# QuantEcon/dynamic_factor_models

Hardware: AMD Instinct MI355X
Metric: Kalman-smoother passes/sec, N=200 T=500 r=8 panel (higher is better)
Workload: dtype f64; 1 GPU; BASELINE configs[1]: synthetic panel N=200 T=500 r=8, batch=1024 replicates per GPU, one full Kalman-smoother pass per step, balanced; N=200, T=500, r=8, batch_per_gpu=1024, global_batch=1024, mode=pass, parallelism=replicate-sharded x1

## Files before the change

dynamic_factor_models_amd/csrc/dfm_cov8.h:

```cpp
#pragma once
#include "dfm_cov.h"
#include "dfm_grid.h"

namespace dfm {

constexpr int kCov8TileDoubles = 8 * kTileStride<8>;
constexpr int kCov8ScratchDoubles = 5 * kCov8TileDoubles + 64;
constexpr int kCov8Keep = 8;

struct Cov8Dst {
    double* tab;
    int tab_cap;
    double* tab_over;
    double* stead;
    double* PT;
    double* xi0;
    double* llc;
    int* E;
    int* fill;
    double* PsInf;
    double* SP11; double* SU; double* P0s;
};

template <int R, int NLEV, int KEEP>
__device__ __forceinline__ void cov_grid(const FastArgs& a, int b, double Cel, double ldfull, double* wsm, const Cov8Dst& o,
                                         Grid<R>& G) {
    constexpr int TS = kTileStride<R>, RR = R * R, RT = R * kTileStride<R>;
    const int lane = G.l, i = G.i, j = G.j;
    double* L0 = wsm;
    double* L1 = L0 + RT;
    double* LPT = L1 + RT;
    double* LJ = LPT + RT;
    const int T = a.T, r = a.r;
    const bool diag = (i == j);
    const size_t mo = (size_t)b * RR + lane;

    const double Ael = a.A[mo];
    double Qi = a.Q[mo];
    double Omf = a.P0[mo];
    const double mu0c = a.mu0[(size_t)b * R + j];
    const double detQ = G.sweep_inverse(Qi);
    const double detP0 = G.sweep_inverse(Omf);
    L0[TS * i + j] = Qi;
    L1[TS * j + i] = Ael;
    G.sync();
    const double PsiT = dot_rows<R>(L0, L1, i, j);
    G.sync();
    LPT[TS * i + j] = PsiT;
    L0[TS * j + i] = PsiT;
    G.sync();
    const double Phi = dot_rows<R>(L0, L1, i, j);
    double q0;
    {
        const double xi0r = G.sum_j(Omf * mu0c);
        if (j == 0) o.xi0[i] = xi0r;
        double part = diag ? mu0c * xi0r : 0.0;
        part = G.sum_j(part);
        q0 = G.sum_i(part);
    }
    G.sync();

    LogProd detprod;
    double detM_last = 1.0;
    int E = 0;
    double Zk[KEEP], Jk[KEEP];
#pragma unroll
    for (int u = 0; u < KEEP; ++u) { Zk[u] = 0.0; Jk[u] = 0.0; }
    double Zlast = 0.0, Jlast = 0.0, Glast = 0.0;
    for (int e = 0;; ++e) {
        double Z = Omf + Phi;
        const double detM = G.sweep_inverse(Z);
        L0[TS * i + j] = Z;
        G.sync();
        const double Jr = dot_rows<R>(L0, LPT, i, j);
        L1[TS * j + i] = Jr;
        G.sync();
        const double tmp = dot_rows<R>(LPT, L1, i, j);
        const double Gm = dot_rows<R>(LPT, L0, i, j);
        const double Omf_new = (Qi - tmp) + Cel;
        const bool gsame = G.all_true(close_enough(Omf_new, Omf));
        double* te = (e < o.tab_cap ? o.tab : o.tab_over) + (size_t)e * 3 * RR;
        te[lane] = Z; te[RR + lane] = Jr; te[2 * RR + lane] = Gm;
#pragma unroll
        for (int u = 0; u < KEEP; ++u) {
            Zk[u] = (u == e) ? Z : Zk[u];
            Jk[u] = (u == e) ? Jr : Jk[u];
        }
        Zlast = Z; Jlast = Jr; Glast = Gm;
        E = e + 1;
        detprod.mul(detM);
        detM_last = detM;
        Omf = Omf_new;
        G.sync();
        if (gsame || e + 1 >= T) break;
    }
    const int ts = E - 1;

    double Ps = Omf;
    const double detOmT = G.sweep_inverse(Ps);
    o.PT[lane] = Ps;
    if (lane == 0) {
        const double sum_ldz = -(detprod.log_value() + (double)(T - E) * log(detM_last));
        const double LD = log(detOmT) + log(detP0) + (double)T * log(detQ) - sum_ldz;
        o.llc[0] = (double)a.N * (double)T * kLog2PiF + (double)T * ldfull + LD + q0;
        o.E[0] = E;
    }

    const int npr = r * (r + 1) / 2;
    const bool pout = a.P_smooth != nullptr && i < r && j <= i;
    double* prow = a.P_smooth ? a.P_smooth + (size_t)b * T * npr + i * (i + 1) / 2 + j : nullptr;
    auto emit = [&](int trow, double P) { if (pout) prow[(size_t)trow * npr] = P; };
    emit(T - 1, Ps);
    double SP = Ps, SU = 0.0;
    int fill_lo = 0, fill_hi = 0;
    int t = T - 1, cur_e = -2;
    double Zc = 0.0, Jc = 0.0;
    while (t >= 0) {
        const int e = t < ts ? t : ts;
        if (e != cur_e) {
            if (e == ts) {
                Zc = Zlast; Jc = Jlast;
            } else if (e < KEEP) {
#pragma unroll
                for (int u = 0; u < KEEP; ++u) {
                    Zc = (u == e) ? Zk[u] : Zc;
                    Jc = (u == e) ? Jk[u] : Jc;
                }
            } else {
                const double* te = (e < o.tab_cap ? o.tab : o.tab_over) + (size_t)e * 3 * RR;
                Zc = te[lane]; Jc = te[RR + lane];
            }
            cur_e = e;
            LJ[TS * i + j] = Jc;
        }
        L0[TS * i + j] = Ps;
        G.sync();
        const double U = dot_rows<R>(L0, LJ, i, j);
        L1[TS * j + i] = U;
        G.sync();
        const double Psn = Zc + dot_rows<R>(LJ, L1, i, j);
        const bool gsame = G.all_true(close_enough(Psn, Ps));
        const bool skip = (e == ts && t > ts && gsame);
        const int plo = ts >= 1 ? ts : 1;
        const double cu = skip ? (double)(t - ts + 1) : 1.0;
        const double cp = (t >= 1 ? 1.0 : 0.0) + (skip ? (double)(t - plo) : 0.0);
        SU = fma(cu, U, SU);
        SP = fma(cp, Psn, SP);
        if (t >= 1) emit(t - 1, Psn);
        if ((t == 0 || (skip && ts == 0)) && o.P0s) o.P0s[lane] = Psn;
        if (skip) {
            o.PsInf[lane] = Psn;
            fill_lo = plo - 1;
            fill_hi = t - 1;
            t = ts - 1;
        } else {
            t -= 1;
        }
        Ps = Psn;
        G.sync();
    }
    if (lane == 0) { o.fill[0] = fill_lo; o.fill[1] = fill_hi; }
    if (o.SP11) { o.SP11[lane] = SP; o.SU[lane] = SU; }

    {
        const double Zs = Zlast, Js = Jlast, Gs = Glast;
        o.stead[lane] = Zs;
        o.stead[2 * RR + lane] = Gs;
        o.stead[1 * RR + lane] = Js;
        double MG = Gs, MJ = Js;
        auto square2 = [&]() {
            L0[TS * i + j] = MG;
            L1[TS * j + i] = MG;
            LPT[TS * i + j] = MJ;
            LJ[TS * j + i] = MJ;
            G.sync();
            MG = dot_rows<R>(L0, L1, i, j);
            MJ = dot_rows<R>(LPT, LJ, i, j);
            G.sync();
        };
        for (int l = 1; l < a.L; l <<= 1) square2();
#pragma unroll 1
        for (int k = 0; k < NLEV; ++k) {
            o.stead[(3 + k) * RR + lane] = MG;
            o.stead[(3 + NLEV + k) * RR + lane] = MJ;
            if (k + 1 < NLEV) square2();
        }
    }
}

template <int NLEV>
__device__ __forceinline__ void cov_wave8(const FastArgs& a, int b, double Cel, double ldfull, double* wsm, const Cov8Dst& o,
                                          int lane) {
    Grid<8> G;
    G.l = lane; G.i = lane >> 3; G.j = lane & 7; G.prow = nullptr; G.red = nullptr; G.tt = nullptr;
    cov_grid<8, NLEV, kCov8Keep>(a, b, Cel, ldfull, wsm, o, G);
}

template <int NDR>
__device__ __forceinline__ double gram_wave8(const double* __restrict__ Lg, const double* __restrict__ Rg, int N, int lane,
                                             double* Cs) {
    constexpr int R = 8;
    double W[NDR][2][R];
    bool own[NDR][2];
    double ld = 0.0;
#pragma unroll
    for (int q = 0; q < NDR; ++q)
#pragma unroll
        for (int e = 0; e < 2; ++e) {
            const int c = 2 * lane + 128 * q + e;
            own[q][e] = c < N;
            const int cc = own[q][e] ? c : N - 1;
            const double rv = own[q][e] ? Rg[cc] : 1.0;
            const double ri = own[q][e] ? 1.0 / rv : 0.0;
            ld += log(rv);
#pragma unroll
            for (int k = 0; k < R; ++k) W[q][e][k] = Lg[(size_t)cc * R + k] * ri;
        }
    c_chunk<R, NDR, 0, 18, true>(W, Lg, own, lane, Cs);
    c_chunk<R, NDR, 18, 18, true>(W, Lg, own, lane, Cs);
    return wave_allsum(ld);
}

}
```

dynamic_factor_models_amd/csrc/pass_fused.hip:

```cpp
#include <stdlib.h>
#include <string.h>

#include <type_traits>

#include "dfm_cov8.h"
#include "dfm_gram.h"
#include "dfm_kernels.h"
#include "dfm_scan.h"

#ifndef DFM_DMA_MOD
#define DFM_DMA_MOD ""
#endif

namespace dfm {

namespace {

using lds_char_ptr_f = __attribute__((address_space(3))) char*;

__device__ __forceinline__ void dma16f(const void* gsrc, unsigned lds_dst, bool nt) {
    unsigned keep;
    if (nt) {
        asm volatile(
            "s_mov_b32 %0, m0\n\t"
            "s_mov_b32 m0, %2\n\t"
            "s_nop 0\n\t"
            "global_load_lds_dwordx4 %1, off nt\n\t"
            "s_mov_b32 m0, %0"
            : "=&s"(keep)
            : "v"(gsrc), "s"(lds_dst)
            : "memory");
    } else {
        asm volatile(
            "s_mov_b32 %0, m0\n\t"
            "s_mov_b32 m0, %2\n\t"
            "s_nop 0\n\t"
            "global_load_lds_dwordx4 %1, off" DFM_DMA_MOD "\n\t"
            "s_mov_b32 m0, %0"
            : "=&s"(keep)
            : "v"(gsrc), "s"(lds_dst)
            : "memory");
    }
}
template <int K>
__device__ __forceinline__ void wait_vmf() {
    asm volatile("s_waitcnt vmcnt(%0)" ::"i"(K) : "memory");
}
__device__ __forceinline__ void wait_lgkmf() { asm volatile("s_waitcnt lgkmcnt(0)" ::: "memory"); }

constexpr int kPfR = 8;
#ifndef DFM_PF_ECAP
#define DFM_PF_ECAP 8
#endif
constexpr int kPfEcap = DFM_PF_ECAP;
constexpr int kPfNst = stead_mats(kPfR);
constexpr int kPfNlev = scan_levels(kPfR);
constexpr int kPfScanWaves = kScanThreads / 64;
constexpr int kPfMaxCov = 2;
#ifndef DFM_PF_DEFER
#define DFM_PF_DEFER 4
#endif
constexpr int kPfDeferDefault = DFM_PF_DEFER;
constexpr int kPfMaxWaves = 12;
constexpr int kPfMaxThreads = 64 * kPfMaxWaves;
constexpr unsigned kPfLdsLimit = 160u * 1024u;

constexpr int kFBtReady = 0;
constexpr int kFScanDone = 2;
constexpr int kFCovDone = 3;
constexpr int kFScanBar = 5;
constexpr int kFAbort = 6;
constexpr int kFTabReady = 7;
constexpr int kFScanArrive = 8;
constexpr int kFStreamWaits = 9;
constexpr int kFCount = 64;

constexpr int kMiscXi0 = 0, kMiscLlc = 8, kMiscE = 9, kMiscVec = 16, kMiscRed = 32, kMiscSsum = 40 ,
              kMiscPs = 56 , kMiscWtr = 92 , kMiscDoubles = 92 + kPfEcap * 8;

__host__ __device__ inline unsigned pf_slot_bytes(int N) {
    unsigned sb = (unsigned)N * 8u;
    while ((sb & 255u) != 64u && (sb & 255u) != 192u) sb += 16u;
    return sb;
}

__device__ __forceinline__ unsigned ld_flag(const unsigned* f) {
    return __builtin_amdgcn_readfirstlane(__hip_atomic_load(f, __ATOMIC_RELAXED, __HIP_MEMORY_SCOPE_WORKGROUP));
}
__device__ __forceinline__ bool pf_wait_ge(const unsigned* f, unsigned target, unsigned* abortf) {
    unsigned spins = 0;
    for (;;) {
        if ((int)(ld_flag(f) - target) >= 0) break;
        __builtin_amdgcn_s_sleep(2);
        if ((++spins & 255u) == 0) {
            if (ld_flag(abortf) != 0) return false;
            if (spins > (1u << 23)) {
                __hip_atomic_store(abortf, 1u, __ATOMIC_RELAXED, __HIP_MEMORY_SCOPE_WORKGROUP);
                return false;
            }
        }
    }
    __builtin_amdgcn_fence(__ATOMIC_ACQUIRE, "workgroup");
    return true;
}
__device__ __forceinline__ void pf_signal(unsigned* f, int lane) {
    __builtin_amdgcn_fence(__ATOMIC_RELEASE, "workgroup");
    if (lane == 0) __hip_atomic_fetch_add(f, 1u, __ATOMIC_RELAXED, __HIP_MEMORY_SCOPE_WORKGROUP);
}

// ... 2 lines not shown
    unsigned* abortf;
    unsigned gen;
    int lane;
    __device__ __forceinline__ void operator()() {
        gen += kPfScanWaves;
        __builtin_amdgcn_fence(__ATOMIC_RELEASE, "workgroup");
        if (lane == 0) __hip_atomic_fetch_add(ctr, 1u, __ATOMIC_RELAXED, __HIP_MEMORY_SCOPE_WORKGROUP);
        unsigned spins = 0;
        while ((int)(ld_flag(ctr) - gen) < 0) {
            __builtin_amdgcn_s_sleep(1);
            if ((++spins & 1023u) == 0) {
                if (ld_flag(abortf) != 0) break;
                if (spins > (1u << 23)) { __hip_atomic_store(abortf, 1u, __ATOMIC_RELAXED, __HIP_MEMORY_SCOPE_WORKGROUP); break; }
            }
        }
        __builtin_amdgcn_fence(__ATOMIC_ACQUIRE, "workgroup");
    }
};

__device__ __forceinline__ double ld_dev(const double* p) { return __hip_atomic_load(p, __ATOMIC_RELAXED, __HIP_MEMORY_SCOPE_AGENT); }
__device__ __forceinline__ int ld_dev(const int* p) { return __hip_atomic_load(p, __ATOMIC_RELAXED, __HIP_MEMORY_SCOPE_AGENT); }

}

__device__ __forceinline__ void pf_fill_rows(double* Prep, int lo, int hi, int npr, const double* ps, int lane, int w, int nw) {
    const int per = (hi - lo + nw - 1) / nw;
    const int a0 = lo + w * per;
    const int a1 = a0 + per < hi ? a0 + per : hi;
    if (a1 <= a0) return;
    double* base = Prep + (size_t)a0 * npr;
    const unsigned n = (unsigned)(a1 - a0) * (unsigned)npr;
    const unsigned peel = ((reinterpret_cast<size_t>(base) & 15) != 0) ? 1u : 0u;
    if (peel && lane == 0) base[0] = ps[0];
    const unsigned npair = (n - peel) / 2;
    const unsigned step = 128u % (unsigned)npr;
    unsigned k = peel + 2u * lane;
    unsigned v = k % (unsigned)npr;
    for (unsigned p = lane; p < npair; p += 64) {
        const unsigned v1 = (v + 1 == (unsigned)npr) ? 0u : v + 1;
        *reinterpret_cast<double2*>(base + k) = make_double2(ps[v], ps[v1]);
        k += 128u;
        v += step;
        if (v >= (unsigned)npr) v -= (unsigned)npr;
    }
    if (((n - peel) & 1u) != 0 && lane == 0) base[n - 1] = ps[(n - 1) % (unsigned)npr];
}

struct PfLds {
    unsigned flags;
    unsigned smat;
    unsigned ctab;
    unsigned misc;
    unsigned covws;
    unsigned sa, sb;
    unsigned bt;
    unsigned bt_stride;
    unsigned ring;
    unsigned total;
    int nsw, ncov, nbuf;
    int nt;
};

#if defined(DFM_DIAG) || defined(DFM_PF_FALLBACK_LDS)
template <class Sync>
__device__ __forceinline__ void scan_lds(const FastArgs& a, int b, int tid, double* bt, const double* s_tab, const double* tab_over,
                                         const double* s_mat, const double* xi0p, const double* llcp, int E, double* s_a,
                                         double* s_b, double* s_vec, double* s_red, const double* ssum, int nseg, Sync& sync,
                                         double* pslot) {
    auto mark = [&](int k) {
        if (pslot && tid == 0) pslot[k] = (double)__builtin_amdgcn_s_memrealtime();
    };
    constexpr int R = kPfR;
    constexpr int NG = kScanThreads / R;
    constexpr int NLEV = kPfNlev;
    constexpr int NST = kPfNst;
    const int c = tid / R, i = tid % R;
    const int T = a.T, r = a.r, L = a.L;
    const int ts = E - 1;
    const int nst = ts < kPfEcap ? ts : kPfEcap;
    double* fout = a.f_smooth + (size_t)b * T * r;
    double xi = xi0p[i];
    const int clast = (T - 1 - ts) / L;
    const int cmax = c | (64 / R - 1);
    const int t0f = ts + c * L;
    const int t0b = T - 1 - c * L;
    const bool fullf = (ts + (cmax + 1) * L) <= T;
    const bool fullb = (T - (cmax + 1) * L) >= ts;
    double cur[kPF];
    double dot = 0.0;

    if (ts > 0) {
        if (tid < 64) {
            for (int t = 0; t < ts; ++t) {
                double Zp[R], Gp[R];
                const double* ent = t < nst ? s_tab + (size_t)t * 3 * R * R : tab_over + (size_t)t * 3 * R * R;
                load_xperm<R>(Zp, ent, i);
                load_xperm<R>(Gp, ent + 2 * R * R, i);
                const double btv = bt[t * R + i];
                const double w = matvec_x<R>(Zp, xi);
                wave_lds_sync();
                if (c == 0) {
                    dot = fma(xi, w, dot);
                    bt[t * R + i] = w;
                }
                xi = matvec_x<R>(Gp, xi, btv);
            }
            if (c == 0) s_vec[i] = xi;
        }
        sync();
        xi = s_vec[i];
        sync();
    }
    mark(1);

    {
// ... 38 lines not shown
        const double e = fullb ? chunk_run<R, true, 0>(Jp, Jp, 0.0, cur, bt, t0b, -1, L, ts, T, i, nullptr, dummy, nullptr, r)
                               : chunk_run<R, false, 0>(Jp, Jp, 0.0, cur, bt, t0b, -1, L, ts, T, i, nullptr, dummy, nullptr, r);
        if (fullb) chunk_prefetch<R, true>(cur, bt, t0b, -1, L, ts, T, i);
        else chunk_prefetch<R, false>(cur, bt, t0b, -1, L, ts, T, i);
        mark(5);
        const double s = carry_scan<R, NG>(e, fT, s_mat + (size_t)(3 + NLEV) * R * R, c, i, s_a, s_b, true, sync);
        mark(6);
        const double v = fullb ? chunk_run<R, true, 2>(Jp, Jp, s, cur, bt, t0b, -1, L, ts, T, i, nullptr, dummy, fout, r)
                               : chunk_run<R, false, 2>(Jp, Jp, s, cur, bt, t0b, -1, L, ts, T, i, nullptr, dummy, fout, r);
        if (c == clast) s_vec[R + i] = v;
        sync();
        fb = s_vec[R + i];
    }

    mark(7);
    if (tid < 64) {
        double v = fb;
        for (int t = ts - 1; t >= 0; --t) {
            double Jp[R];
            load_xperm<R>(Jp, (t < nst ? s_tab + (size_t)t * 3 * R * R : tab_over + (size_t)t * 3 * R * R) + R * R, i);
            const double wt = bt[t * R + i];
            v = matvec_x<R>(Jp, v, wt);
            if (c == 0 && t >= 1 && i < r) fout[(size_t)(t - 1) * r + i] = v;
        }
        if (a.f0s && c == 0) a.f0s[(size_t)b * R + i] = v;
    }

    mark(8);
#pragma unroll
    for (int off = 32; off >= 1; off >>= 1) dot += __shfl_xor(dot, off, kWave);
    if ((tid & 63) == 0) s_red[tid >> 6] = dot;
    sync();
    if (tid == 0) {
        double d = 0.0, sq = 0.0;
#pragma unroll
        for (int w = 0; w < kScanThreads / 64; ++w) d += s_red[w];
        for (int w = 0; w < nseg; ++w) sq += ssum[w];
        a.loglik[b] = -0.5 * (llcp[0] + sq - d);
    }
}

#endif

constexpr int kRegL = 16;

template <class Sync, class Prio>
__device__ __forceinline__ void scan_reg(const FastArgs& a, int b, int tid, const double* bt, const double* s_tab, const double* s_mat,
                                         const double* xi0p, const double* llcp, int E, double* sE, double* sEb, double* s_red,
                                         const double* ssum, int nseg, Sync& sync, unsigned* arrive, unsigned arrive_last,
                                         unsigned* scan_done, unsigned done_value, double* wtr, Prio&& prio, double* pslot) {
    auto mark = [&](int k) {
        if (pslot && tid == 0) pslot[k] = (double)__builtin_amdgcn_s_memrealtime();
    };
    constexpr int R = kPfR, NLEV = kPfNlev, NST = kPfNst, LM = kRegL;
    const int c = tid / R, i = tid % R, lane = tid & 63;
    const int T = a.T, r = a.r, L = a.L;
    const int ts = E - 1;
    double* fout = a.f_smooth + (size_t)b * T * r;
    const int clast = (T - ts - 1) / L;
    const int t0 = ts + c * L;
    const int Lc = (T - t0) < L ? (T - t0) : L;
    const int wlo = __builtin_amdgcn_readfirstlane(c & ~7);
    double dot = 0.0;

    double xi = xi0p[i];
#pragma unroll
    for (int t = 0; t < kPfEcap; ++t) {
        if (t < ts) {
            double Zp[R], Gp[R];
            const double* ent = s_tab + (size_t)t * 3 * R * R;
            load_xperm<R>(Zp, ent, i);
            load_xperm<R>(Gp, ent + 2 * R * R, i);
            const double btv = bt[t * R + i];
            const double w = matvec_x<R>(Zp, xi);
            if (c == 0) {
                dot = fma(xi, w, dot);
                wtr[t * R + i] = w;
            }
            xi = matvec_x<R>(Gp, xi, btv);
        }
    }
    mark(1);

    double u[LM];
#pragma unroll
    for (int j = 0; j < LM; ++j) {
        u[j] = 0.0;
        if (j < L) {
            const bool ok = j < Lc;
            const int tc = ok ? t0 + j : T - 1;
            const double x = bt[tc * R + i];
            u[j] = ok ? x : 0.0;
        }
    }
    double Gp[R];
    load_xperm<R>(Gp, s_mat + 2 * R * R, i);
    {
        double e = 0.0;
#pragma unroll
        for (int j = 0; j < LM; ++j) {
            if (j < L) {
                const double vn = matvec_x<R>(Gp, e, u[j]);
                e = (j < Lc) ? vn : e;
            }
        }
        sE[c * R + i] = e;
    }
    mark(2);
    sync();
    prio();
    double v = xi;
    {
        double ML[R];
        load_xperm<R>(ML, s_mat + 3 * R * R, i);
        for (int k0 = 0; k0 <= wlo; k0 += 8) {
            double ek[8];
#pragma unroll
            for (int q = 0; q < 8; ++q) ek[q] = sE[(k0 + q) * R + i];
#pragma unroll
            for (int q = 0; q < 8; ++q) {
                const double vn = matvec_x<R>(ML, v, ek[q]);
                v = (k0 + q < c) ? vn : v;
            }
        }
    }
    mark(3);
    {
        double Zp[R];
        load_xperm<R>(Zp, s_mat, i);
#pragma unroll
        for (int j = 0; j < LM; ++j) {
            if (j < L) {
                const bool ok = j < Lc;
                const double w = matvec_x<R>(Zp, v);
                const double vn = matvec_x<R>(Gp, v, u[j]);
                dot = ok ? fma(v, w, dot) : dot;
                u[j] = w;
                v = ok ? vn : v;
            }
        }
    }
    mark(4);
    double Jp[R];
    load_xperm<R>(Jp, s_mat + R * R, i);
    double eb;
    {
        double PTp[R];
        load_xperm<R>(PTp, s_mat + NST * R * R, i);
        const double fT = matvec_x<R>(PTp, v);
        const bool top = (c == clast);
        if (top) {
            dot = fma(v, fT, dot);
            if (i < r) fout[(size_t)(T - 1) * r + i] = fT;
        }
        eb = top ? fT : 0.0;
#pragma unroll
        for (int j = LM - 1; j >= 0; --j) {
            if (j < L) {
                const bool ok = j < Lc;
                const double vn = matvec_x<R>(Jp, eb, u[j]);
                eb = ok ? vn : eb;
                const int t = t0 + j;
                if (top && ok && t >= 1 && i < r) fout[(size_t)(t - 1) * r + i] = eb;
            }
        }
        sEb[c * R + i] = eb;
    }
    mark(5);
    sync();
    prio();
    double vb = 0.0;
    if (wlo < clast) {
        double JL[R];
        load_xperm<R>(JL, s_mat + (size_t)(3 + NLEV) * R * R, i);
        vb = sEb[clast * R + i];
        for (int k0 = clast - 1; k0 > wlo; k0 -= 8) {
            double ek[8];
#pragma unroll
            for (int q = 0; q < 8; ++q) { const int k = k0 - q; ek[q] = sEb[(k > 0 ? k : 0) * R + i]; }
#pragma unroll
            for (int q = 0; q < 8; ++q) {
                const double vn = matvec_x<R>(JL, vb, ek[q]);
                vb = (k0 - q > c) ? vn : vb;
            }
        }
    }
    mark(6);
    {
        const bool below = c < clast;
#pragma unroll
        for (int j = LM - 1; j >= 0; --j) {
            if (j < L) {
                vb = matvec_x<R>(Jp, vb, u[j]);
                const int t = t0 + j;
                if (below && t >= 1 && i < r) fout[(size_t)(t - 1) * r + i] = vb;
            }
        }
        vb = below ? vb : eb;
    }
    mark(7);
    if (tid < 64) {
        double vt = vb;
#pragma unroll
        for (int t = kPfEcap - 1; t >= 0; --t) {
            if (t < ts) {
                double Jt[R];
                load_xperm<R>(Jt, s_tab + (size_t)t * 3 * R * R + R * R, i);
                vt = matvec_x<R>(Jt, vt, wtr[t * R + (tid & 7)]);
                if (c == 0 && t >= 1 && i < r) fout[(size_t)(t - 1) * r + i] = vt;
            }
        }
        if (a.f0s && c == 0) {
            int ii = tid & 7;
            asm volatile("" : "+v"(ii));
            a.f0s[(size_t)b * R + ii] = vt;
        }
    }
    mark(8);
#pragma unroll
    for (int off = 32; off >= 1; off >>= 1) dot += __shfl_xor(dot, off, kWave);
    if (lane == 0) s_red[tid >> 6] = dot;
    __builtin_amdgcn_fence(__ATOMIC_RELEASE, "workgroup");
    unsigned before = 0;
    if (lane == 0) before = __hip_atomic_fetch_add(arrive, 1u, __ATOMIC_RELAXED, __HIP_MEMORY_SCOPE_WORKGROUP);
    before = __builtin_amdgcn_readfirstlane(before);
    if (before + 1u == arrive_last) {
        __builtin_amdgcn_fence(__ATOMIC_ACQUIRE, "workgroup");
        if (lane == 0) {
            double d = 0.0, sq = 0.0;
#pragma unroll
            for (int w = 0; w < kPfScanWaves; ++w) d += s_red[w];
            for (int w = 0; w < nseg; ++w) sq += ssum[w];
            a.loglik[b] = -0.5 * (llcp[0] + sq - d);
            __hip_atomic_store(scan_done, done_value, __ATOMIC_RELEASE, __HIP_MEMORY_SCOPE_WORKGROUP);
        }
    }
}

__device__ __forceinline__ void scan_seq(const FastArgs& a, int b, int tid, double* bt, const double* s_tab, const double* tab_over,
                                         const double* s_mat, const double* xi0p, const double* llcp, int E, const double* ssum, int nseg,
                                         unsigned* arrive, unsigned arrive_last, unsigned* scan_done, unsigned done_value) {
    constexpr int R = kPfR, NST = kPfNst;
    const int lane = tid & 63, i = tid % R, c = tid / R;
    const int T = a.T, r = a.r;
    const int ts = E - 1;
    const int nst = ts < kPfEcap ? ts : kPfEcap;
    double dot = 0.0;
    if (tid < 64) {
        double* fout = a.f_smooth + (size_t)b * T * r;
        double xi = xi0p[i];
        double Zs[R], Gs[R];
        load_xperm<R>(Zs, s_mat, i);
        load_xperm<R>(Gs, s_mat + 2 * R * R, i);
        for (int t = 0; t < T; ++t) {
            double Zp[R], Gp[R];
            if (t < ts) {
                const double* ent = t < nst ? s_tab + (size_t)t * 3 * R * R : tab_over + (size_t)t * 3 * R * R;
                load_xperm<R>(Zp, ent, i);
                load_xperm<R>(Gp, ent + 2 * R * R, i);
            } else {
#pragma unroll
                for (int k = 0; k < R; ++k) { Zp[k] = Zs[k]; Gp[k] = Gs[k]; }
            }
            const double btv = bt[t * R + i];
            const double w = matvec_x<R>(Zp, xi);
            wave_lds_sync();
            if (c == 0) { dot = fma(xi, w, dot); bt[t * R + i] = w; }
            xi = matvec_x<R>(Gp, xi, btv);
        }
        double PTp[R];
        load_xperm<R>(PTp, s_mat + NST * R * R, i);
        double v = matvec_x<R>(PTp, xi);
        if (c == 0) {
            dot = fma(xi, v, dot);
            if (i < r) fout[(size_t)(T - 1) * r + i] = v;
        }
        wave_lds_sync();
        double Js[R];
        load_xperm<R>(Js, s_mat + R * R, i);
        for (int t = T - 1; t >= 0; --t) {
            double Jp[R];
            if (t < ts) load_xperm<R>(Jp, (t < nst ? s_tab + (size_t)t * 3 * R * R : tab_over + (size_t)t * 3 * R * R) + R * R, i);
            else {
#pragma unroll
                for (int k = 0; k < R; ++k) Jp[k] = Js[k];
            }
            v = matvec_x<R>(Jp, v, bt[t * R + i]);
            if (c == 0 && t >= 1 && i < r) fout[(size_t)(t - 1) * r + i] = v;
        }
        if (a.f0s && c == 0) a.f0s[(size_t)b * R + i] = v;
        dot = (c == 0) ? dot : 0.0;
#pragma unroll
        for (int off = 4; off >= 1; off >>= 1) dot += __shfl_xor(dot, off, kWave);
        if (lane == 0) {
            double sq = 0.0;
// ... 65 lines not shown
        Cs[(4 + K) * R + 4 * h + q] = D1;
    }
    return wave_allsum(ld);
}

template <int STEPS, int NDR>
__global__ __launch_bounds__(kPfMaxThreads) void pass_fused_kernel(CollapseArgs a, FastArgs fa, unsigned SB, PfLds ly) {
    constexpr int R = kPfR;
    constexpr int NB = 2, NS = 4 * NB;
    constexpr int CS = 8;
    constexpr int NQ = NDR;
    extern __shared__ __attribute__((aligned(16))) char smem[];
    const int tid_wg = threadIdx.x;
    const int lane = tid_wg & 63;
    const int wave = __builtin_amdgcn_readfirstlane(tid_wg >> 6);
    const int nsw = ly.nsw, ncov = ly.ncov, nbuf = ly.nbuf;
    const bool dma_nt = ly.nt != 0;
    unsigned* flags = reinterpret_cast<unsigned*>(smem + ly.flags);
    double* misc = reinterpret_cast<double*>(smem + ly.misc);
    double* bt0 = reinterpret_cast<double*>(smem + ly.bt);
    const int N = a.N, T = a.T, B = a.B;
    const int G = (int)gridDim.x;
    const int nrep_wg = (B - (int)blockIdx.x + G - 1) / G;
#ifdef DFM_DIAG
    const int ndefer = (fa.P_smooth == nullptr) ? 0 : (((fa.abl >> 12) & 7) ? ((fa.abl >> 12) & 7) - 1 : kPfDeferDefault);
#else
    const int ndefer = (fa.P_smooth == nullptr) ? 0 : kPfDeferDefault;
#endif

    if (tid_wg < kFCount) flags[tid_wg] = 0u;
    __syncthreads();

#ifdef DFM_DIAG
    const bool prof = (fa.abl & 256) != 0 && a.scol != nullptr && T >= 40;
    auto stamp = [&](int bb, int slot) {
        if (prof && lane == 0) a.scol[(size_t)bb * T + slot] = (double)__builtin_amdgcn_s_memrealtime();
    };

    if (prof) {
        const unsigned hw = __builtin_amdgcn_s_getreg((31 << 11) | 4);
        for (int bb = (int)blockIdx.x; bb < B; bb += G) {
            if (lane == 0) a.scol[(size_t)bb * T + 40 + wave] = (double)hw;
        }
    }
#else
    constexpr bool prof = false;
    auto stamp = [](int, int) {};
#endif

    if (wave < nsw) {
        const unsigned rowB = (unsigned)N * 8u;
        const int K = lane >> 4, blk = (lane >> 2) & 3, q = lane & 3;
        const int g = blk >> 1, h = blk & 1;
        int tq = (T + nsw - 1) / nsw;
        {
            unsigned gg = rowB & 127u;
            gg = gg == 0 ? 128u : (gg & (~gg + 1u));
            const int m = (int)(128u / gg);
            tq = ((tq + m - 1) / m) * m;
        }
        const int ta = (wave * tq < T) ? wave * tq : T;
        const int tb = (ta + tq < T) ? ta + tq : T;
        const int nrows = tb - ta;
        const int nblk = (nrows + 3) / 4;
        const unsigned ringB = NS * SB;
        const char* ring = smem + ly.ring + (size_t)wave * ringB;
        const unsigned ring_lds =
            __builtin_amdgcn_readfirstlane((unsigned)(size_t)(lds_char_ptr_f)(smem)) + ly.ring + (unsigned)wave * ringB;
        const unsigned lane16 = 16u * lane;
        bool pact[NDR];
#pragma unroll
        for (int p = 0; p < NDR; ++p) pact[p] = lane16 + 1024u * p < rowB;
        const unsigned lane_off = (unsigned)q * SB + (unsigned)(4 * g + K) * 8u;
        const bool tail_clamp = (STEPS - 1) * CS + 4 * g + K >= N;
        const unsigned last_off = tail_clamp ? (unsigned)q * SB + (unsigned)(N - 1) * 8u : lane_off + (unsigned)(STEPS - 1) * (CS * 8u);
        const int nrep = (B - (int)blockIdx.x + G - 1) / G;
        const int gtot = nrep * nblk;

        double Bw[STEPS];
        double rown[NQ][2];
        auto issue_block = [&](int jj, int k, int bslot) {
            const char* seg = reinterpret_cast<const char*>(a.panel + ((size_t)((int)blockIdx.x + jj * G) * T + ta) * N);
#pragma unroll
            for (int rr = 0; rr < 4; ++rr) {
                int ri = 4 * k + rr;
                ri = ri < nrows ? ri : nrows - 1;
                const char* src = seg + (size_t)ri * rowB + lane16;
                const unsigned dst = __builtin_amdgcn_readfirstlane(ring_lds + (unsigned)(bslot * 4 + rr) * SB);
#pragma unroll
                for (int p = 0; p < NDR; ++p) {
                    if (pact[p]) dma16f(src + 1024 * p, dst + 1024u * p, dma_nt);
                }
            }
        };
        auto load_weights = [&](int bb) {
            const double* __restrict__ Lq = a.Lam + (size_t)bb * N * R + (4 * g + K) * R + 4 * h + q;
            const double* __restrict__ Rq = a.Rv + (size_t)bb * N + (4 * g + K);
            const int clast = tail_clamp ? N - 1 : (STEPS - 1) * CS + 4 * g + K;
            double rv[STEPS];
#pragma unroll
            for (int s = 0; s + 1 < STEPS; ++s) {
                Bw[s] = Lq[s * CS * R];
                rv[s] = Rq[s * CS];
            }
            Bw[STEPS - 1] = a.Lam[(size_t)bb * N * R + (size_t)clast * R + 4 * h + q];
            rv[STEPS - 1] = a.Rv[(size_t)bb * N + clast];
            const double* __restrict__ Rg = a.Rv + (size_t)bb * N;
#pragma unroll
            for (int jq = 0; jq < NQ; ++jq)
#pragma unroll
                for (int e = 0; e < 2; ++e) {
                    const int c = 2 * lane + 128 * jq + e;
                    rown[jq][e] = Rg[c < N ? c : N - 1];
                }
            __builtin_amdgcn_sched_barrier(0);
// ... 52 lines not shown
                    const char* pq = blkbase + lane16;
                    double2 xq[4][NQ];
#pragma unroll
                    for (int rr = 0; rr < 4; ++rr)
#pragma unroll
                        for (int jq = 0; jq < NQ; ++jq)
                            xq[rr][jq] = pact[jq] ? *reinterpret_cast<const double2*>(pq + (unsigned)rr * SB + 1024u * jq)
                                                  : make_double2(0.0, 0.0);
                    wait_lgkmf();
                    if (ij < nrep) { issue_block(ij, ik, bslot); advance_issue(); }
                    double D = 0.0, D2 = 0.0;
#pragma unroll
                    for (int s = 0; s < STEPS; ++s) {
                        if ((s & 1) == 0) D = __builtin_amdgcn_mfma_f64_4x4x4f64(xa[s], Bw[s], D, 0, 0, 0);
                        else D2 = __builtin_amdgcn_mfma_f64_4x4x4f64(xa[s], Bw[s], D2, 0, 0, 0);
                    }
                    D += D2;
#pragma unroll
                    for (int rr = 0; rr < 4; ++rr) {
                        if (full || r0 + rr < nrows) {
#pragma unroll
                            for (int jq = 0; jq < NQ; ++jq) {
                                qa[jq][0] = fma(xq[rr][jq].x, xq[rr][jq].x, qa[jq][0]);
                                qa[jq][1] = fma(xq[rr][jq].y, xq[rr][jq].y, qa[jq][1]);
                            }
                        }
                    }
                    D += xor_lane<8>(D);
                    const double hi = xor_lane<1>(D);
                    const int t = ta + r0 + K;
                    if (g == 0 && (q & 1) == 0 && t < tb)
                        *reinterpret_cast<double2*>(&bt[(size_t)t * R + 4 * h + q]) = make_double2(D, hi);
                    bslot = (bslot + 1 == NB) ? 0 : bslot + 1;
                }
                double sp = 0.0;
#pragma unroll
                for (int jq = 0; jq < NQ; ++jq)
#pragma unroll
                    for (int e = 0; e < 2; ++e) sp = fma(qa[jq][e], rown[jq][e], sp);
                sp = wave_allsum(sp);
                if (lane == 0) {
                    misc[kMiscSsum + buf * 8 + wave] = sp;
                    if (sp != sp) atomicOr(a.status, 1);
                }
                wait_lgkmf();
                __builtin_amdgcn_wave_barrier();
                if (lane == 0) __hip_atomic_fetch_add(flags + kFBtReady + buf, 1u, __ATOMIC_RELAXED, __HIP_MEMORY_SCOPE_WORKGROUP);
                if (wave == 0) stamp(b, 2);
                if (wave == nsw - 1) stamp(b, 3);
                stamp(b, 24 + wave);
            }
            if (ndefer > 0) {
                wait_vmf<0>();
                const int nact = (T + tq - 1) / tq;
                const int npr = fa.r * (fa.r + 1) / 2;
                double* ps = reinterpret_cast<double*>(const_cast<char*>(ring));
                for (int j = (nrep - ndefer > 0 ? nrep - ndefer : 0); j < nrep; ++j) {
                    const int b = (int)blockIdx.x + j * G;
                    if (!pf_wait_ge(flags + kFTabReady, (unsigned)(j + 1), flags + kFAbort)) break;
                    const int flo = __builtin_amdgcn_readfirstlane(ld_dev(fa.fill + 2 * b));
                    const int fhi = __builtin_amdgcn_readfirstlane(ld_dev(fa.fill + 2 * b + 1));
                    if (fhi <= flo) continue;
                    int ri = 0;
                    const int lv = lane < npr ? lane : 0;
                    while ((ri + 1) * (ri + 2) / 2 <= lv) ++ri;
                    const double psv = ld_dev(fa.PsInf + (size_t)b * 64 + ri * R + (lv - ri * (ri + 1) / 2));
                    wave_lds_sync();
                    if (lane < npr) ps[lane] = psv;
                    wave_lds_sync();
                    pf_fill_rows(fa.P_smooth + (size_t)b * T * npr, flo, fhi, npr, ps, lane, wave, nact);
                }
            }
        } else {
            for (int j = 0; j < nrep; ++j) {
                const int buf = nbuf == 2 ? (j & 1) : 0;
                if (j >= nbuf) {
                    if (!pf_wait_ge(flags + kFScanDone, (unsigned)(j - nbuf + 1), flags + kFAbort)) return;
                }
                if (lane == 0) {
                    misc[kMiscSsum + buf * 8 + wave] = 0.0;
                }
                pf_signal(flags + kFBtReady + buf, lane);
            }
        }
    } else if (wave < nsw + ncov) {
        const int cw = wave - nsw;
        double* ws = reinterpret_cast<double*>(smem + ly.covws) + (size_t)cw * kCov8ScratchDoubles;
        double* Cs = ws + 5 * kCov8TileDoubles;
        __builtin_amdgcn_s_setprio(2);
        for (int b = (int)blockIdx.x + cw * G; b < B; b += ncov * G) {
            stamp(b, 6);
            const double ld = gram_mfma8<STEPS, NDR>(fa.Lam + (size_t)b * N * R, fa.Rv + (size_t)b * N, N, lane, Cs,
                                                     prof ? a.scol + (size_t)b * T + 36 : nullptr);
            wave_lds_sync();
            const double Cel = 0.5 * (Cs[lane] + Cs[(lane & 7) * 8 + (lane >> 3)]);
            wave_lds_sync();
            __builtin_amdgcn_sched_barrier(0);
            Cov8Dst o;
            o.tab = fa.tab + (size_t)b * T * 3 * 64; o.tab_cap = T; o.tab_over = o.tab;
            o.stead = fa.stead + (size_t)b * kPfNst * 64;
            o.PT = fa.PT + (size_t)b * 64; o.xi0 = fa.xi0 + (size_t)b * 8; o.llc = fa.llc + b; o.E = fa.E + b;
            o.fill = fa.fill + 2 * b; o.PsInf = fa.PsInf + (size_t)b * 64;
            o.SP11 = fa.SP11 ? fa.SP11 + (size_t)b * 64 : nullptr;
            o.SU = fa.SP11 ? fa.SU + (size_t)b * 64 : nullptr;
            o.P0s = fa.SP11 ? fa.P0s + (size_t)b * 64 : nullptr;
            stamp(b, 7);
            cov_wave8<kPfNlev>(fa, b, Cel, ld, ws, o, lane);
            wave_lds_sync();
            stamp(b, 8);
            pf_signal(flags + kFCovDone + cw, lane);
        }
    } else if (wave == nsw + ncov) {
        double* s_mat = reinterpret_cast<double*>(smem + ly.smat);
        double* s_tab = reinterpret_cast<double*>(smem + ly.ctab);
        double* s_ps = misc + kMiscPs;
        const int nfix0 = kPfEcap < T ? kPfEcap : T;
        __builtin_amdgcn_s_setprio(1);
        int b = blockIdx.x;
        for (int j = 0; b < B; b += G, ++j) {
            if (!pf_wait_ge(flags + kFCovDone + (j % ncov), (unsigned)(j / ncov + 1), flags + kFAbort)) break;
            stamp(b, 4);
            const double* stead = fa.stead + (size_t)b * kPfNst * 64;
            const double* tab = fa.tab + (size_t)b * T * 3 * 64;
            double ms[kPfNst + 1], mt[kPfEcap * 3];
#pragma unroll
            for (int k = 0; k < kPfNst; ++k) ms[k] = stead[k * 64 + lane];
            ms[kPfNst] = fa.PT[(size_t)b * 64 + lane];
#pragma unroll
            for (int k = 0; k < kPfEcap * 3; ++k) mt[k] = (k < nfix0 * 3) ? tab[k * 64 + lane] : 0.0;
            const int Ev = ld_dev(fa.E + b);
            const double xiv = ld_dev(fa.xi0 + (size_t)b * R + (lane & 7));
            const double llv = ld_dev(fa.llc + b);
            const int npr = fa.r * (fa.r + 1) / 2;
            int flo = 0, fhi = 0;
            double psv = 0.0;
            if (fa.P_smooth) {
                flo = ld_dev(fa.fill + 2 * b);
                fhi = ld_dev(fa.fill + 2 * b + 1);
                int ri = 0;
                const int lv = lane < npr ? lane : 0;
                while ((ri + 1) * (ri + 2) / 2 <= lv) ++ri;
                psv = ld_dev(fa.PsInf + (size_t)b * 64 + ri * R + (lv - ri * (ri + 1) / 2));
            }
            __builtin_amdgcn_sched_barrier(0);
            const int E = __builtin_amdgcn_readfirstlane(Ev);
            const double xl = lane < R ? xiv : llv;
            const int fill_lo = __builtin_amdgcn_readfirstlane(flo), fill_hi = __builtin_amdgcn_readfirstlane(fhi);
            if (j >= 1) {
                if (!pf_wait_ge(flags + kFScanDone, (unsigned)j, flags + kFAbort)) break;
            }
#pragma unroll
            for (int k = 0; k <= kPfNst; ++k) s_mat[k * 64 + lane] = ms[k];
#pragma unroll
            for (int k = 0; k < kPfEcap * 3; ++k) s_tab[k * 64 + lane] = mt[k];
            if (lane <= R) misc[kMiscXi0 + lane] = xl;
            if (lane == 0) misc[kMiscE] = (double)E;
            pf_signal(flags + kFTabReady, lane);
            stamp(b, 5);
            if (fill_hi > fill_lo && j < nrep_wg - ndefer) {
                if (lane < npr) s_ps[lane] = psv;
                wave_lds_sync();
                pf_fill_rows(fa.P_smooth + (size_t)b * T * npr, fill_lo, fill_hi, npr, s_ps, lane, 0, 1);
                wave_lds_sync();
            }
        }
    } else if (wave < nsw + ncov + 1 + kPfScanWaves) {
        const int tid = tid_wg - 64 * (nsw + ncov + 1);
        double* s_mat = reinterpret_cast<double*>(smem + ly.smat);
        double* s_tab = reinterpret_cast<double*>(smem + ly.ctab);
        double* s_a = reinterpret_cast<double*>(smem + ly.sa);
        double* s_b = reinterpret_cast<double*>(smem + ly.sb);
        PfScanSync sync{flags + kFScanBar, flags + kFAbort, 0u, lane};
#ifdef DFM_DIAG
        const bool use_reg = fa.L <= kRegL && (fa.abl & 512) == 0;
        const int prio_mode = (fa.abl & 1024) ? 1 : (fa.abl & 2048) ? 2 : 0;
#else
#ifndef DFM_PF_PRIO_MODE
#define DFM_PF_PRIO_MODE 0
#endif
        constexpr int prio_mode = DFM_PF_PRIO_MODE;
#endif
        auto set_prio = [&](int j) {
            const bool hot = prio_mode == 1 || (prio_mode == 0 && (j == 0 || ld_flag(flags + kFStreamWaits) != 0)) ||
                             (prio_mode == 3 && ld_flag(flags + kFStreamWaits) != 0) || (prio_mode == 4 && j == 0);
            if (hot) __builtin_amdgcn_s_setprio(3);
            else __builtin_amdgcn_s_setprio(0);
        };
        __builtin_amdgcn_s_setprio(3);
        int b = blockIdx.x;
        for (int j = 0; b < B; b += G, ++j) {
            const int buf = nbuf == 2 ? (j & 1) : 0;
            double* bt = bt0 + (size_t)buf * ly.bt_stride;
            if (tid == 0) stamp(b, 10);
            if (!pf_wait_ge(flags + kFTabReady, (unsigned)(j + 1), flags + kFAbort)) break;
            if (tid == 0) stamp(b, 11);
            if (!pf_wait_ge(flags + kFBtReady + buf, (unsigned)(nsw * (j / nbuf + 1)), flags + kFAbort)) break;
            if (tid == 0) stamp(b, 12);
            set_prio(j);
            const int E = __builtin_amdgcn_readfirstlane((int)misc[kMiscE]);
#ifdef DFM_DIAG
            if (!use_reg) {
                scan_lds(fa, b, tid, bt, s_tab, fa.tab + (size_t)b * T * 3 * 64, s_mat, misc + kMiscXi0, misc + kMiscLlc, E, s_a, s_b,
                         misc + kMiscVec, misc + kMiscRed, misc + kMiscSsum + buf * 8, nsw, sync,
                         (prof && tid == 0) ? a.scol + (size_t)b * T + 13 : nullptr);
                sync();
                if (lane == 0) __hip_atomic_fetch_add(flags + kFScanArrive, 1u, __ATOMIC_RELAXED, __HIP_MEMORY_SCOPE_WORKGROUP);
                if (tid == 0) {
                    __hip_atomic_store(flags + kFScanDone, (unsigned)(j + 1), __ATOMIC_RELEASE, __HIP_MEMORY_SCOPE_WORKGROUP);
                    stamp(b, 22);
                }
                continue;
            }
            double* const pslot = (prof && tid == 0) ? a.scol + (size_t)b * T + 13 : nullptr;
#else
            double* const pslot = nullptr;
#endif
            if (E - 1 <= kPfEcap) {
                scan_reg(fa, b, tid, bt, s_tab, s_mat, misc + kMiscXi0, misc + kMiscLlc, E, s_a, s_b, misc + kMiscRed,
                         misc + kMiscSsum + buf * 8, nsw, sync, flags + kFScanArrive, (unsigned)(kPfScanWaves * (j + 1)),
                         flags + kFScanDone, (unsigned)(j + 1), misc + kMiscWtr, [&]() { set_prio(j); }, pslot);
            } else {
#ifdef DFM_PF_FALLBACK_LDS
                scan_lds(fa, b, tid, bt, s_tab, fa.tab + (size_t)b * T * 3 * 64, s_mat, misc + kMiscXi0, misc + kMiscLlc, E, s_a, s_b,
                         misc + kMiscVec, misc + kMiscRed, misc + kMiscSsum + buf * 8, nsw, sync, nullptr);
                sync();
                if (lane == 0) __hip_atomic_fetch_add(flags + kFScanArrive, 1u, __ATOMIC_RELAXED, __HIP_MEMORY_SCOPE_WORKGROUP);
                if (tid == 0) __hip_atomic_store(flags + kFScanDone, (unsigned)(j + 1), __ATOMIC_RELEASE, __HIP_MEMORY_SCOPE_WORKGROUP);
                continue;
#endif
                scan_seq(fa, b, tid, bt, s_tab, fa.tab + (size_t)b * T * 3 * 64, s_mat, misc + kMiscXi0, misc + kMiscLlc, E,
                         misc + kMiscSsum + buf * 8, nsw, flags + kFScanArrive, (unsigned)(kPfScanWaves * (j + 1)),
                         flags + kFScanDone, (unsigned)(j + 1));
            }
            if (tid == 0) stamp(b, 22);
        }
    }
    if (lane == 0 && ld_flag(flags + kFAbort) != 0) atomicOr(a.status, 4);
}

static PfLds pf_layout(int T, int N, int nsw, int ncov, int nbuf) {
    PfLds l;
    unsigned off = 0;
    auto take = [&](unsigned bytes) { const unsigned at = off; off += (bytes + 255u) & ~255u; return at; };
    l.flags = take(kFCount * 4);
    l.smat = take((kPfNst + 1) * 64 * 8);
    l.ctab = take(kPfEcap * 3 * 64 * 8);
    l.misc = take(kMiscDoubles * 8);
    l.covws = take((unsigned)ncov * kCov8ScratchDoubles * 8);
    l.sa = take(32 * 8 * 8);
    l.sb = take(32 * 8 * 8);
    const unsigned btb = (unsigned)((T + 3) / 4 * 4) * 8 * 8;
    l.bt_stride = ((btb + 255u) & ~255u) / 8;
    l.bt = take(l.bt_stride * 8 * (unsigned)nbuf);
    l.ring = take((unsigned)nsw * 8u * pf_slot_bytes(N));
    l.total = off;
    l.nsw = nsw; l.ncov = ncov; l.nbuf = nbuf; l.nt = 0;
    return l;
}

static PfLds pf_pick(int T, int N, int want_nsw, int want_ncov) {
    int ncov = want_ncov > 0 ? want_ncov : kPfMaxCov;
    if (ncov > kPfMaxCov) ncov = kPfMaxCov;
    int cap = kPfMaxWaves - kPfScanWaves - 1 - ncov;
    if (want_nsw <= 0) want_nsw = 4;
    if (want_nsw < cap) cap = want_nsw;
    while (cap > 1 && T / cap < 8) --cap;
    for (int nbuf = 2; nbuf >= 1; --nbuf) {
        for (int nsw = cap; nsw >= (nbuf == 2 ? (cap < 3 ? cap : 3) : 1); --nsw) {
            const PfLds l = pf_layout(T, N, nsw, ncov, nbuf);
            if (l.total <= kPfLdsLimit) return l;
        }
    }
    PfLds none = pf_layout(T, N, 1, ncov, 1);
    return none;
}

int pass_fused_pick_nsw(int T, int N, int want) { return pf_pick(T, N, want, 0).nsw; }

bool pass_fused_supported(int Rpad, int T, int N) {
    if (Rpad != 8 || !collapse_mfma_supported(8, N)) return false;
    if (T < 2) return false;
#ifndef DFM_DIAG
    if (fast_chunk_len(8, T) > kRegL) return false;
#endif
    return pf_pick(T, N, 0, 0).total <= kPfLdsLimit;
}

template <int STEPS, int NDR>
static hipError_t launch_pf_one(const CollapseArgs& a, const FastArgs& fa, int nsw, int ncov, int num_cu, hipStream_t s) {
    PfLds ly = pf_pick(a.T, a.N, nsw, ncov);
    if (ly.total > kPfLdsLimit) return hipErrorInvalidValue;
    ly.nt = stream_nt_hint((size_t)a.B * a.T * a.N * sizeof(double)) ? 1 : 0;
    static LdsOptIn attr_done;
    if (!attr_done) {
        hipError_t e = hipFuncSetAttribute(reinterpret_cast<const void*>(&pass_fused_kernel<STEPS, NDR>),
                                           hipFuncAttributeMaxDynamicSharedMemorySize, (int)kPfLdsLimit);
        if (e != hipSuccess) return e;
        attr_done = true;
    }
    const int grid = a.B < num_cu ? a.B : num_cu;
    const int nwaves = ly.nsw + ly.ncov + 1 + kPfScanWaves;
// ... 109 lines not shown
```

Before: 4.946 million passes/s.

## Stage covariance results through LDS park and drop global round-trip via staging wave

New measurement: 5.034 million passes/s, median of 6. 1.02x the previous value.

```diff
diff --git a/dynamic_factor_models_amd/csrc/dfm_cov8.h b/dynamic_factor_models_amd/csrc/dfm_cov8.h
--- a/dynamic_factor_models_amd/csrc/dfm_cov8.h
+++ b/dynamic_factor_models_amd/csrc/dfm_cov8.h
@@ -20,11 +20,13 @@
     int* fill;
     double* PsInf;
     double* SP11; double* SU; double* P0s;
+    double* gpark = nullptr;
+    double* PT_g = nullptr;
 };
 
 template <int R, int NLEV, int KEEP>
 __device__ __forceinline__ void cov_grid(const FastArgs& a, int b, double Cel, double ldfull, double* wsm, const Cov8Dst& o,
-                                         Grid<R>& G) {
+                                         Grid<R>& G, double (&Zk)[KEEP], double (&Jk)[KEEP]) {
     constexpr int TS = kTileStride<R>, RR = R * R, RT = R * kTileStride<R>;
     const int lane = G.l, i = G.i, j = G.j;
     double* L0 = wsm;
@@ -63,7 +65,6 @@
     LogProd detprod;
     double detM_last = 1.0;
     int E = 0;
-    double Zk[KEEP], Jk[KEEP];
 #pragma unroll
     for (int u = 0; u < KEEP; ++u) { Zk[u] = 0.0; Jk[u] = 0.0; }
     double Zlast = 0.0, Jlast = 0.0, Glast = 0.0;
@@ -79,8 +80,12 @@
         const double Gm = dot_rows<R>(LPT, L0, i, j);
         const double Omf_new = (Qi - tmp) + Cel;
         const bool gsame = G.all_true(close_enough(Omf_new, Omf));
-        double* te = (e < o.tab_cap ? o.tab : o.tab_over) + (size_t)e * 3 * RR;
-        te[lane] = Z; te[RR + lane] = Jr; te[2 * RR + lane] = Gm;
+        if (o.gpark && e < KEEP) {
+            o.gpark[(size_t)e * RR + lane] = Gm;
+        } else {
+            double* te = (e < o.tab_cap ? o.tab : o.tab_over) + (size_t)e * 3 * RR;
+            te[lane] = Z; te[RR + lane] = Jr; te[2 * RR + lane] = Gm;
+        }
 #pragma unroll
         for (int u = 0; u < KEEP; ++u) {
             Zk[u] = (u == e) ? Z : Zk[u];
@@ -99,6 +104,7 @@
     double Ps = Omf;
     const double detOmT = G.sweep_inverse(Ps);
     o.PT[lane] = Ps;
+    if (o.PT_g) o.PT_g[lane] = Ps;
     if (lane == 0) {
         const double sum_ldz = -(detprod.log_value() + (double)(T - E) * log(detM_last));
         const double LD = log(detOmT) + log(detP0) + (double)T * log(detQ) - sum_ldz;
@@ -187,13 +193,25 @@
         }
     }
 }
-
+template <int R, int NLEV, int KEEP>
+__device__ __forceinline__ void cov_grid(const FastArgs& a, int b, double Cel, double ldfull, double* wsm, const Cov8Dst& o,
+                                         Grid<R>& G) {
+    double Zk[KEEP], Jk[KEEP];
+    cov_grid<R, NLEV, KEEP>(a, b, Cel, ldfull, wsm, o, G, Zk, Jk);
+}
+
+template <int NLEV>
+__device__ __forceinline__ void cov_wave8(const FastArgs& a, int b, double Cel, double ldfull, double* wsm, const Cov8Dst& o,
+                                          int lane, double (&Zk)[kCov8Keep], double (&Jk)[kCov8Keep]) {
+    Grid<8> G;
+    G.l = lane; G.i = lane >> 3; G.j = lane & 7; G.prow = nullptr; G.red = nullptr; G.tt = nullptr;
+    cov_grid<8, NLEV, kCov8Keep>(a, b, Cel, ldfull, wsm, o, G, Zk, Jk);
+}
 template <int NLEV>
 __device__ __forceinline__ void cov_wave8(const FastArgs& a, int b, double Cel, double ldfull, double* wsm, const Cov8Dst& o,
                                           int lane) {
-    Grid<8> G;
-    G.l = lane; G.i = lane >> 3; G.j = lane & 7; G.prow = nullptr; G.red = nullptr; G.tt = nullptr;
-    cov_grid<8, NLEV, kCov8Keep>(a, b, Cel, ldfull, wsm, o, G);
+    double Zk[kCov8Keep], Jk[kCov8Keep];
+    cov_wave8<NLEV>(a, b, Cel, ldfull, wsm, o, lane, Zk, Jk);
 }
 
 template <int NDR>
diff --git a/dynamic_factor_models_amd/csrc/pass_fused.hip b/dynamic_factor_models_amd/csrc/pass_fused.hip
--- a/dynamic_factor_models_amd/csrc/pass_fused.hip
+++ b/dynamic_factor_models_amd/csrc/pass_fused.hip
@@ -55,6 +55,17 @@
 constexpr int kPfEcap = DFM_PF_ECAP;
 constexpr int kPfNst = stead_mats(kPfR);
 constexpr int kPfNlev = scan_levels(kPfR);
+static_assert(kPfEcap == kCov8Keep, "the covariance wave keeps Z_e, J_e of exactly the staged transient steps in registers");
+#ifdef DFM_DIAG
+constexpr int kPfNlevTab = kPfNlev;
+#else
+constexpr int kPfNlevTab = 1;
+#endif
+constexpr int kPfGL = 3;
+constexpr int kPfJL = 3 + kPfNlevTab;
+constexpr int kPfNstTab = 3 + 2 * kPfNlevTab;
+constexpr int kParkG = (kPfNstTab + 1) * 64, kParkXi0 = kParkG + kPfEcap * 64, kParkLlc = kParkXi0 + 8, kParkE = kParkLlc + 1,
+              kParkDoubles = kParkXi0 + 16;
 constexpr int kPfScanWaves = kScanThreads / 64;
 constexpr int kPfMaxCov = 2;
 #ifndef DFM_PF_DEFER
@@ -163,6 +174,7 @@
     unsigned ctab;
     unsigned misc;
     unsigned covws;
+    unsigned park;
     unsigned sa, sb;
     unsigned bt;
     unsigned bt_stride;
@@ -172,6 +184,9 @@
     int nt;
 };
 
+#if defined(DFM_PF_FALLBACK_LDS) && !defined(DFM_DIAG)
+#error "scan_lds needs every carry power in the table set: build with -DDFM_DIAG"
+#endif
 #if defined(DFM_DIAG) || defined(DFM_PF_FALLBACK_LDS)
 template <class Sync>
 __device__ __forceinline__ void scan_lds(const FastArgs& a, int b, int tid, double* bt, const double* s_tab, const double* tab_over,
@@ -316,7 +331,7 @@
     auto mark = [&](int k) {
         if (pslot && tid == 0) pslot[k] = (double)__builtin_amdgcn_s_memrealtime();
     };
-    constexpr int R = kPfR, NLEV = kPfNlev, NST = kPfNst, LM = kRegL;
+    constexpr int R = kPfR, NST = kPfNstTab, LM = kRegL;
     const int c = tid / R, i = tid % R, lane = tid & 63;
     const int T = a.T, r = a.r, L = a.L;
     const int ts = E - 1;
@@ -376,7 +391,7 @@
     double v = xi;
     {
         double ML[R];
-        load_xperm<R>(ML, s_mat + 3 * R * R, i);
+        load_xperm<R>(ML, s_mat + kPfGL * R * R, i);
         for (int k0 = 0; k0 <= wlo; k0 += 8) {
             double ek[8];
 #pragma unroll
@@ -436,7 +451,7 @@
     double vb = 0.0;
     if (wlo < clast) {
         double JL[R];
-        load_xperm<R>(JL, s_mat + (size_t)(3 + NLEV) * R * R, i);
+        load_xperm<R>(JL, s_mat + (size_t)kPfJL * R * R, i);
         vb = sEb[clast * R + i];
         for (int k0 = clast - 1; k0 > wlo; k0 -= 8) {
             double ek[8];
@@ -504,7 +519,7 @@
 __device__ __forceinline__ void scan_seq(const FastArgs& a, int b, int tid, double* bt, const double* s_tab, const double* tab_over,
                                          const double* s_mat, const double* xi0p, const double* llcp, int E, const double* ssum, int nseg,
                                          unsigned* arrive, unsigned arrive_last, unsigned* scan_done, unsigned done_value) {
-    constexpr int R = kPfR, NST = kPfNst;
+    constexpr int R = kPfR, NST = kPfNstTab;
     const int lane = tid & 63, i = tid % R, c = tid / R;
     const int T = a.T, r = a.r;
     const int ts = E - 1;
@@ -676,15 +691,19 @@
         const unsigned rowB = (unsigned)N * 8u;
         const int K = lane >> 4, blk = (lane >> 2) & 3, q = lane & 3;
         const int g = blk >> 1, h = blk & 1;
-        int tq = (T + nsw - 1) / nsw;
+        int unit;
         {
             unsigned gg = rowB & 127u;
             gg = gg == 0 ? 128u : (gg & (~gg + 1u));
             const int m = (int)(128u / gg);
-            tq = ((tq + m - 1) / m) * m;
-        }
-        const int ta = (wave * tq < T) ? wave * tq : T;
-        const int tb = (ta + tq < T) ? ta + tq : T;
+            unit = m < 4 ? 4 : m;
+        }
+        const int nunit = (T + unit - 1) / unit;
+        const int ubase = nunit / nsw, urem = nunit % nsw;
+        const int ua = wave * ubase + (wave < urem ? wave : urem);
+        const int ub = ua + ubase + (wave < urem ? 1 : 0);
+        const int ta = (ua * unit < T) ? ua * unit : T;
+        const int tb = (ub * unit < T) ? ub * unit : T;
         const int nrows = tb - ta;
         const int nblk = (nrows + 3) / 4;
         const unsigned ringB = NS * SB;
@@ -843,7 +862,7 @@
             }
             if (ndefer > 0) {
                 wait_vmf<0>();
-                const int nact = (T + tq - 1) / tq;
+                const int nact = nunit < nsw ? nunit : nsw;
                 const int npr = fa.r * (fa.r + 1) / 2;
                 double* ps = reinterpret_cast<double*>(const_cast<char*>(ring));
                 for (int j = (nrep - ndefer > 0 ? nrep - ndefer : 0); j < nrep; ++j) {
@@ -878,8 +897,12 @@
         const int cw = wave - nsw;
         double* ws = reinterpret_cast<double*>(smem + ly.covws) + (size_t)cw * kCov8ScratchDoubles;
         double* Cs = ws + 5 * kCov8TileDoubles;
+        double* park = reinterpret_cast<double*>(smem + ly.park) + (size_t)cw * kParkDoubles;
+        double* s_mat = reinterpret_cast<double*>(smem + ly.smat);
+        double* s_tab = reinterpret_cast<double*>(smem + ly.ctab);
         __builtin_amdgcn_s_setprio(2);
-        for (int b = (int)blockIdx.x + cw * G; b < B; b += ncov * G) {
+        int j = cw;
+        for (int b = (int)blockIdx.x + cw * G; b < B; b += ncov * G, j += ncov) {
             stamp(b, 6);
             const double ld = gram_mfma8<STEPS, NDR>(fa.Lam + (size_t)b * N * R, fa.Rv + (size_t)b * N, N, lane, Cs,
                                                      prof ? a.scol + (size_t)b * T + 36 : nullptr);
@@ -888,72 +911,61 @@
             wave_lds_sync();
             __builtin_amdgcn_sched_barrier(0);
             Cov8Dst o;
-            o.tab = fa.tab + (size_t)b * T * 3 * 64; o.tab_cap = T; o.tab_over = o.tab;
-            o.stead = fa.stead + (size_t)b * kPfNst * 64;
-            o.PT = fa.PT + (size_t)b * 64; o.xi0 = fa.xi0 + (size_t)b * 8; o.llc = fa.llc + b; o.E = fa.E + b;
+            o.tab = nullptr; o.tab_cap = 0; o.tab_over = fa.tab + (size_t)b * T * 3 * 64;
+            o.gpark = park + kParkG;
+            o.stead = park;
+            o.PT = park + kPfNstTab * 64; o.xi0 = park + kParkXi0; o.llc = park + kParkLlc;
+            o.E = reinterpret_cast<int*>(park + kParkE);
             o.fill = fa.fill + 2 * b; o.PsInf = fa.PsInf + (size_t)b * 64;
             o.SP11 = fa.SP11 ? fa.SP11 + (size_t)b * 64 : nullptr;
             o.SU = fa.SP11 ? fa.SU + (size_t)b * 64 : nullptr;
             o.P0s = fa.SP11 ? fa.P0s + (size_t)b * 64 : nullptr;
+            o.PT_g = fa.SP11 ? fa.PT + (size_t)b * 64 : nullptr;
             stamp(b, 7);
-            cov_wave8<kPfNlev>(fa, b, Cel, ld, ws, o, lane);
+            double Zk[kCov8Keep], Jk[kCov8Keep];
+            cov_wave8<kPfNlevTab>(fa, b, Cel, ld, ws, o, lane, Zk, Jk);
             wave_lds_sync();
             stamp(b, 8);
-            pf_signal(flags + kFCovDone + cw, lane);
-        }
-    } else if (wave == nsw + ncov) {
-        double* s_mat = reinterpret_cast<double*>(smem + ly.smat);
-        double* s_tab = reinterpret_cast<double*>(smem + ly.ctab);
-        double* s_ps = misc + kMiscPs;
-        const int nfix0 = kPfEcap < T ? kPfEcap : T;
-        __builtin_amdgcn_s_setprio(1);
-        int b = blockIdx.x;
-        for (int j = 0; b < B; b += G, ++j) {
-            if (!pf_wait_ge(flags + kFCovDone + (j % ncov), (unsigned)(j / ncov + 1), flags + kFAbort)) break;
-            stamp(b, 4);
-            const double* stead = fa.stead + (size_t)b * kPfNst * 64;
-            const double* tab = fa.tab + (size_t)b * T * 3 * 64;
-            double ms[kPfNst + 1], mt[kPfEcap * 3];
-#pragma unroll
-            for (int k = 0; k < kPfNst; ++k) ms[k] = stead[k * 64 + lane];
-            ms[kPfNst] = fa.PT[(size_t)b * 64 + lane];
-#pragma unroll
-            for (int k = 0; k < kPfEcap * 3; ++k) mt[k] = (k < nfix0 * 3) ? tab[k * 64 + lane] : 0.0;
-            const int Ev = ld_dev(fa.E + b);
-            const double xiv = ld_dev(fa.xi0 + (size_t)b * R + (lane & 7));
-            const double llv = ld_dev(fa.llc + b);
-            const int npr = fa.r * (fa.r + 1) / 2;
-            int flo = 0, fhi = 0;
-            double psv = 0.0;
-            if (fa.P_smooth) {
-                flo = ld_dev(fa.fill + 2 * b);
-                fhi = ld_dev(fa.fill + 2 * b + 1);
-                int ri = 0;
-                const int lv = lane < npr ? lane : 0;
-                while ((ri + 1) * (ri + 2) / 2 <= lv) ++ri;
-                psv = ld_dev(fa.PsInf + (size_t)b * 64 + ri * R + (lv - ri * (ri + 1) / 2));
-            }
-            __builtin_amdgcn_sched_barrier(0);
-            const int E = __builtin_amdgcn_readfirstlane(Ev);
-            const double xl = lane < R ? xiv : llv;
-            const int fill_lo = __builtin_amdgcn_readfirstlane(flo), fill_hi = __builtin_amdgcn_readfirstlane(fhi);
             if (j >= 1) {
                 if (!pf_wait_ge(flags + kFScanDone, (unsigned)j, flags + kFAbort)) break;
             }
-#pragma unroll
-            for (int k = 0; k <= kPfNst; ++k) s_mat[k * 64 + lane] = ms[k];
-#pragma unroll
-            for (int k = 0; k < kPfEcap * 3; ++k) s_tab[k * 64 + lane] = mt[k];
-            if (lane <= R) misc[kMiscXi0 + lane] = xl;
-            if (lane == 0) misc[kMiscE] = (double)E;
-            pf_signal(flags + kFTabReady, lane);
+            stamp(b, 4);
+#pragma unroll
+            for (int k = 0; k <= kPfNstTab; ++k) s_mat[k * 64 + lane] = park[k * 64 + lane];
+#pragma unroll
+            for (int e = 0; e < kPfEcap; ++e) {
+                s_tab[(3 * e) * 64 + lane] = Zk[e];
+                s_tab[(3 * e + 1) * 64 + lane] = Jk[e];
+                s_tab[(3 * e + 2) * 64 + lane] = park[kParkG + e * 64 + lane];
+            }
+            if (lane <= R) misc[kMiscXi0 + lane] = park[kParkXi0 + lane];
+            if (lane == 0) misc[kMiscE] = (double)o.E[0];
+            __builtin_amdgcn_fence(__ATOMIC_RELEASE, "workgroup");
+            if (lane == 0) {
+                __hip_atomic_store(flags + kFTabReady, (unsigned)(j + 1), __ATOMIC_RELAXED, __HIP_MEMORY_SCOPE_WORKGROUP);
+                __hip_atomic_fetch_add(flags + kFCovDone + cw, 1u, __ATOMIC_RELAXED, __HIP_MEMORY_SCOPE_WORKGROUP);
+            }
+            wave_lds_sync();
             stamp(b, 5);
-            if (fill_hi > fill_lo && j < nrep_wg - ndefer) {
-                if (lane < npr) s_ps[lane] = psv;
-                wave_lds_sync();
-                pf_fill_rows(fa.P_smooth + (size_t)b * T * npr, fill_lo, fill_hi, npr, s_ps, lane, 0, 1);
-                wave_lds_sync();
-            }
+        }
+    } else if (wave == nsw + ncov) {
+        double* s_ps = misc + kMiscPs;
+        __builtin_amdgcn_s_setprio(1);
+        const int npr = fa.r * (fa.r + 1) / 2;
+        int b = blockIdx.x;
+        for (int j = 0; j < nrep_wg - ndefer && fa.P_smooth != nullptr; b += G, ++j) {
+            if (!pf_wait_ge(flags + kFTabReady, (unsigned)(j + 1), flags + kFAbort)) break;
+            const int fill_lo = __builtin_amdgcn_readfirstlane(ld_dev(fa.fill + 2 * b));
+            const int fill_hi = __builtin_amdgcn_readfirstlane(ld_dev(fa.fill + 2 * b + 1));
+            if (fill_hi <= fill_lo) continue;
+            int ri = 0;
+            const int lv = lane < npr ? lane : 0;
+            while ((ri + 1) * (ri + 2) / 2 <= lv) ++ri;
+            const double psv = ld_dev(fa.PsInf + (size_t)b * 64 + ri * R + (lv - ri * (ri + 1) / 2));
+            if (lane < npr) s_ps[lane] = psv;
+            wave_lds_sync();
+            pf_fill_rows(fa.P_smooth + (size_t)b * T * npr, fill_lo, fill_hi, npr, s_ps, lane, 0, 1);
+            wave_lds_sync();
         }
     } else if (wave < nsw + ncov + 1 + kPfScanWaves) {
         const int tid = tid_wg - 64 * (nsw + ncov + 1);
@@ -1034,10 +1046,11 @@
     unsigned off = 0;
     auto take = [&](unsigned bytes) { const unsigned at = off; off += (bytes + 255u) & ~255u; return at; };
     l.flags = take(kFCount * 4);
-    l.smat = take((kPfNst + 1) * 64 * 8);
+    l.smat = take((kPfNstTab + 1) * 64 * 8);
     l.ctab = take(kPfEcap * 3 * 64 * 8);
     l.misc = take(kMiscDoubles * 8);
     l.covws = take((unsigned)ncov * kCov8ScratchDoubles * 8);
+    l.park = take((unsigned)ncov * kParkDoubles * 8);
     l.sa = take(32 * 8 * 8);
     l.sb = take(32 * 8 * 8);
     const unsigned btb = (unsigned)((T + 3) / 4 * 4) * 8 * 8;
```
